# Banus/pano360

Hardware: AMD Instinct MI355X
Metric: blended megapixels/sec (multiband) (higher is better)
Workload: dtype f32; 1 GPU; cfg3: 32 synthetic 3840x2160 frames per image set, spherical warp + multiband blend L=5, native resolution (MAX_RESOLUTION uncapped); frames=32

## Files before the change

pano360_amd/csrc/blend.hip:

```cpp
#include <stdlib.h>

#include "geom.h"

__global__ __launch_bounds__(256) void ownership_kernel(
    const pano_patch *__restrict__ patches, int n, int H, int W,
    int16_t *__restrict__ owner, uint8_t *__restrict__ valid) {
    const int x = blockIdx.x * 64 + threadIdx.x, y = blockIdx.y * 4 + threadIdx.y;
    if (x >= W || y >= H) return;
    float best = 0.0f;
    int who = -1;
    bool any = false;
    for (int i = 0; i < n; ++i) {
        const pano_patch p = patches[i];
        const int px = x - p.x0, py = y - p.y0;
        if ((unsigned)px >= (unsigned)p.w || (unsigned)py >= (unsigned)p.h) continue;
        const float a = p.planes[3 * (size_t)p.vh * p.vpitch + (size_t)py * p.vpitch + px];
        if (a > best) {
            best = a;
            who = i;
        }
        any |= p.mask[(size_t)py * p.w + px] == 0;
    }
    owner[(size_t)y * W + x] = (int16_t)who;
    valid[(size_t)y * W + x] = any ? 1 : 0;
// ... 383 lines not shown
            s_rng[2] = lo_t; s_rng[3] = hi_t;
        }
        __syncthreads();
        const int tid = wave * 64 + lane;
        const bool keep = tid < listed && alpha_bound(cams + sh.list[tid], s_rng).hi >= 0.0f;
        const unsigned long long bal = __ballot(keep);
        if (lane == 0) s_kept[wave] = __popcll(bal);
        __syncthreads();
        int off = 0;
        for (int w = 0; w < wave; ++w) off += s_kept[w];
        off += __popcll(bal & ((1ull << lane) - 1ull));
        if (keep) s_keep[off] = sh.list[tid];
        ncand = s_kept[0] + s_kept[1] + s_kept[2] + s_kept[3];
        list = s_keep;
        __syncthreads();
    }

    const int x = bx0 + threadIdx.x, y = by0 + threadIdx.y;
    if (x >= xs1 || y >= H) return;
    const double s = sin_t[x], c = cos_t[x], t = tan_p[y];
    float acc[3] = {0.0f, 0.0f, 0.0f}, wsum = 0.0f;
    uint8_t last[3] = {0, 0, 0};
    bool any = false;
    for (int kk = 0; kk < ncand; ++kk) {
        const int k = LINEAR ? kk : ncand - 1 - kk;
        const int i = listed < 0 ? k : __builtin_amdgcn_readfirstlane(list[k]);
        const pano_camera *cam = cams + i;
        const int px = x - cam->x0, py = y - cam->y0;
        if ((unsigned)px >= (unsigned)cam->w || (unsigned)py >= (unsigned)cam->h) continue;
        float fx, fy;
        const int sw = cam->sw, sh_ = cam->sh;
        if (map_pixel(cam->proj, s, c, t, sw, sh_, fx, fy)) continue;
        any = true;
        const Taps tp = make_taps_unmasked(fx, fy, sw, sh_);
        const TapBytes tb = load_taps(cam->frame, sw, tp);
        float rgb[3];
        const float *__restrict__ gl = lut + (size_t)i * 256;
#pragma unroll
        for (int ch = 0; ch < 3; ++ch)
            rgb[ch] = PERCAM ? lerp4(lut_at(gl, tb.v[0][ch]), lut_at(gl, tb.v[1][ch]), lut_at(gl, tb.v[2][ch]),
                                     lut_at(gl, tb.v[3][ch]), tp)
                             : lerp4(lut_at(s_lut, tb.v[0][ch]), lut_at(s_lut, tb.v[1][ch]), lut_at(s_lut, tb.v[2][ch]),
                                     lut_at(s_lut, tb.v[3][ch]), tp);
        if (LINEAR) {
            const float a = alpha_at(cam->hat_x, cam->hat_y, tp);
#pragma unroll
            for (int ch = 0; ch < 3; ++ch) acc[ch] = acc[ch] + rgb[ch] * a;
            wsum = wsum + a;
        } else {
#pragma unroll
            for (int ch = 0; ch < 3; ++ch) last[ch] = (uint8_t)(int)(255.0f * rgb[ch]);
            break;
        }
    }
    const size_t g = ((size_t)y * W + x) * 3;
    if (LINEAR) {
        const float ws = wsum == 0.0f ? 1.0f : wsum;
#pragma unroll
        for (int ch = 0; ch < 3; ++ch)
            mosaic[g + ch] = (uint8_t)(int)(255.0f * __fdiv_rn(acc[ch], ws));
    } else {
        mosaic[g] = last[0];
        mosaic[g + 1] = last[1];
        mosaic[g + 2] = last[2];
    }
    if (valid) valid[(size_t)y * W + x] = any ? 1 : 0;
}

typedef short own8 __attribute__((ext_vector_type(8), aligned(2)));

__device__ __forceinline__ void owned_box_pixel(int o, int x, int y, bool up, bool down, bool left,
                                                bool right, int W, int32_t *__restrict__ boxes,
                                                int stride, uint8_t *__restrict__ marks) {
    if (o < 0) return;
    if (up && marks) marks[(size_t)o * W + x] = 1;
    if (!left && !right) return;
    if (left && up) {
        atomicMin(&boxes[(size_t)stride * o + 0], y);
        atomicMin(&boxes[(size_t)stride * o + 2], x);
    }
    if (left && down) atomicMax(&boxes[(size_t)stride * o + 1], y);
    if (right && up) atomicMax(&boxes[(size_t)stride * o + 3], x);
}

__global__ __launch_bounds__(256) void owned_boxes_kernel(const int16_t *__restrict__ owner,
                                                          int H, int W, int xs0, int xs1,
                                                          int32_t *__restrict__ boxes, int stride,
                                                          uint8_t *__restrict__ marks) {
    const int x8 = xs0 + (blockIdx.x * 64 + threadIdx.x) * 8, y = blockIdx.y * 4 + threadIdx.y;
    if (x8 >= xs1 || y >= H) return;
    const int16_t *row = owner + (size_t)y * W;
    const bool top = y == 0, bottom = y == H - 1;
    if (x8 + 8 <= xs1) {
        const own8 cur = *(const own8 *)(row + x8);
        const own8 upv = top ? cur : *(const own8 *)(row - W + x8);
        const own8 dnv = bottom ? cur : *(const own8 *)(row + W + x8);
        const int before = x8 == xs0 ? -32768 : row[x8 - 1];
        const int after = x8 + 8 == xs1 ? -32768 : row[x8 + 8];
#pragma unroll
        for (int j = 0; j < 8; ++j) {
            const int o = cur[j];
            const int l = j == 0 ? before : cur[j - 1], r = j == 7 ? after : cur[j + 1];
            owned_box_pixel(o, x8 + j, y, top || upv[j] != o, bottom || dnv[j] != o, l != o, r != o,
                            W, boxes, stride, marks);
        }
        return;
    }
    for (int x = x8; x < xs1; ++x) {
        const int o = row[x];
        owned_box_pixel(o, x, y, top || row[x - W] != o, bottom || row[x + W] != o,
                        x == xs0 || row[x - 1] != o, x == xs1 - 1 || row[x + 1] != o, W, boxes,
                        stride, marks);
    }
}

__device__ __forceinline__ uint8_t quant255(float v) { return (uint8_t)(int)(255.0f * v); }

#define IB PANO_INTERIOR_BLOCK

__global__ __launch_bounds__(256) void block_owner_kernel(const int16_t *__restrict__ owner,
                                                          int H, int W, int xs0, int xs1,
                                                          int H8, int W8, int blo, int bhi,
                                                          int16_t *__restrict__ bown) {
    const int bx = blo + blockIdx.x * 64 + threadIdx.x, by = blockIdx.y * 4 + threadIdx.y;
    if (bx >= bhi || by >= H8) return;
    const int x0 = bx * IB, y0 = by * IB;
    int o = -2;
    if (x0 >= xs0 && (x0 + IB < W ? x0 + IB : W) <= xs1) {
        o = owner[(size_t)y0 * W + x0];
        const bool whole = x0 + IB <= W && (W & 1) == 0;
        if (x0 + IB <= W && y0 + IB <= H) {
            static_assert(IB == 4, "one 8-byte load per block row");
            typedef uint64_t u64_any __attribute__((aligned(2)));
            const uint64_t o16 = (uint16_t)o;
            const uint64_t all = o16 | o16 << 16 | o16 << 32 | o16 << 48;
            uint64_t diff = 0;
#pragma unroll
            for (int dy = 0; dy < IB; ++dy)
                diff |= *(const u64_any *)(owner + (size_t)(y0 + dy) * W + x0) ^ all;
            if (diff) o = -2;
        } else
        for (int dy = 0; dy < IB && o != -2; ++dy) {
            const int y = y0 + dy;
            if (y >= H) break;
            if (whole) {
                const uint32_t *q = (const uint32_t *)(owner + (size_t)y * W + x0);
                const uint32_t both = ((uint32_t)(uint16_t)o << 16) | (uint16_t)o;
                uint32_t diff = 0;
#pragma unroll
                for (int k = 0; k < IB / 2; ++k) diff |= q[k] ^ both;
                if (diff) o = -2;
            } else {
                for (int dx = 0; dx < IB; ++dx) {
                    const int x = x0 + dx;
                    if (x >= W) break;
                    if (owner[(size_t)y * W + x] != o) {
                        o = -2;
                        break;
                    }
                }
            }
        }
    }
    bown[(size_t)by * W8 + bx] = (int16_t)o;
}

#define IT_W 64
#define IT_H 16
#define IT_REACH_MAX 20
__device__ __forceinline__ bool agree(int a, int b) { return a == b || a == -3 || b == -3; }

struct LevelReaches {
    int n;
    int reach[PANO_MAX_LEVELS];
};

__global__ __launch_bounds__(256) void interior_tile_kernel(const int16_t *__restrict__ bown,
                                                            int H8, int W8, int reach, int blo,
                                                            int bhi, int ilo, int ihi,
                                                            uint8_t *__restrict__ interior,
                                                            LevelReaches lv,
                                                            uint8_t *__restrict__ classes) {
    __shared__ int16_t s_own[(IT_H + 2 * IT_REACH_MAX) * (IT_W + 2 * IT_REACH_MAX)];
    __shared__ int16_t s_col[IT_H * (IT_W + 2 * IT_REACH_MAX)];
    __shared__ unsigned long long s_vmask[IT_W + 2 * IT_REACH_MAX];
    const int tid = threadIdx.x, lane = tid & 63, wave = tid >> 6;
    const int bx0 = ilo + blockIdx.x * IT_W, by0 = blockIdx.y * IT_H;
    const int tw = IT_W + 2 * reach, th = IT_H + 2 * reach;
    for (int ty = wave; ty < th; ty += 4) {
        const int y = by0 - reach + ty;
        const bool row_in = y >= 0 && y < H8;
        for (int tx = lane; tx < tw; tx += 64) {
            const int x = bx0 - reach + tx;
            s_own[ty * tw + tx] = (row_in && x >= 0 && x < W8)
                                      ? (x >= blo && x < bhi ? bown[(size_t)y * W8 + x] : (int16_t)-2)
                                      : (int16_t)-3;
        }
    }
    __syncthreads();
    for (int tx = tid; tx < tw; tx += 256) {
        unsigned long long m = 0;
        int prev = s_own[tx];
#pragma unroll 8
        for (int ty = 0; ty + 1 < th; ++ty) {
            const int cur = s_own[(ty + 1) * tw + tx];
            m |= (unsigned long long)agree(prev, cur) << ty;
            prev = cur;
        }
        s_vmask[tx] = m;
    }
    __syncthreads();
    int cls[IT_H / 4];
#pragma unroll
    for (int r = 0; r < IT_H / 4; ++r) cls[r] = 0;
    const int nlv = classes ? lv.n : 1;
    for (int q = 0; q < nlv; ++q) {
        const int rq = classes ? lv.reach[q] : reach, off = reach - rq;
        const unsigned long long full = (1ull << (2 * rq)) - 1ull;
        for (int ry = wave; ry < IT_H; ry += 4)
            for (int tx = lane; tx < tw; tx += 64) {
                const int o = s_own[(ry + reach) * tw + tx];
                const bool same = ((s_vmask[tx] >> (ry + off)) & full) == full;
                s_col[ry * tw + tx] = (int16_t)(o >= 0 && !same ? -2 : o);
            }
        __syncthreads();
#pragma unroll
        for (int r = 0; r < IT_H / 4; ++r) {
            const int ry = wave + 4 * r;
            const int16_t *row = s_col + ry * tw;
            const int a0 = row[lane], a1 = row[min(lane + 1, tw - 1)];
            const int b0 = row[min(lane + 64, tw - 1)], b1 = row[min(lane + 65, tw - 1)];
            const unsigned long long lo = __ballot(lane + 1 < tw && agree(a0, a1));
            const unsigned long long hi = __ballot(lane + 65 < tw && agree(b0, b1));
            const int sh = lane + off;
            const unsigned long long win = sh == 0 ? lo
                                           : sh < 64 ? (lo >> sh) | (hi << (64 - sh))
                                                     : hi >> (sh - 64);
            const int o = row[lane + reach];
            if (o >= 0 && (win & full) == full && cls[r] == q) cls[r] = q + 1;
        }
        __syncthreads();
    }
#pragma unroll
    for (int r = 0; r < IT_H / 4; ++r) {
        const int y = by0 + wave + 4 * r, x = bx0 + lane;
        if (y >= H8 || x >= ihi) continue;
        interior[(size_t)y * W8 + x] = cls[r] == nlv ? 1 : 0;
        if (classes) classes[(size_t)y * W8 + x] = (uint8_t)cls[r];
    }
}

struct InteriorArgs {
    const uint8_t *interior;
    int W8;
    const pano_camera *cams;
    const double *sin_t, *cos_t, *tan_p;
    const float *lut;
    const uint8_t *classes;
};

enum { LUT_LDS = 0, LUT_GLOBAL = 1 };

template <int LUT>
__device__ __forceinline__ void shade_interior(const pano_camera *cam, const float *__restrict__ table,
                                               const InteriorArgs &ia, int x, int y, int W,
                                               uint8_t *__restrict__ mosaic,
                                               float *__restrict__ mosaic_f32) {
    if (!cam->frame) return;
    const int sw = cam->sw, sh = cam->sh;
    float fx, fy;
    map_pixel(cam->proj, table_f64(ia.sin_t, x), table_f64(ia.cos_t, x), table_f64(ia.tan_p, y), sw, sh, fx, fy);
    Taps tp = tap_base(fx, fy);
    TapBytes tb;
    if (__ballot(!taps_interior(tp, sw, sh)) == 0ull) {
        tb = load_taps_interior(cam->frame, sw, tp);
    } else {
        tp.x1 = min(tp.x1, sw - 1);
        tp.y1 = min(tp.y1, sh - 1);
        tb = load_taps(cam->frame, sw, tp);
    }
    const size_t g = ((size_t)y * W + x) * 3;
#pragma unroll
    for (int c = 0; c < 3; ++c) {
        float v = lerp4(lut_at(table, tb.v[0][c]), lut_at(table, tb.v[1][c]),
                        lut_at(table, tb.v[2][c]), lut_at(table, tb.v[3][c]), tp);
        v = v < 0.0f ? 0.0f : (v > 1.0f ? 1.0f : v);
        if (mosaic_f32) mosaic_f32[g + c] = v;
        mosaic[g + c] = (uint8_t)(int)(255.0f * v);
    }
}

template <int LUT>
__device__ __forceinline__ void shade_interior_of(int own, const float *__restrict__ table, int stride,
                                                  const InteriorArgs &ia, int x, int y, int W,
                                                  uint8_t *__restrict__ mosaic,
                                                  float *__restrict__ mosaic_f32) {
    const int own_u = __builtin_amdgcn_readfirstlane(own);
    if (__ballot(own != own_u) == 0)
        shade_interior<LUT>(ia.cams + own_u, table + (size_t)own_u * stride, ia, x, y, W, mosaic, mosaic_f32);
    else
        shade_interior<LUT>(ia.cams + own, table + (size_t)own * stride, ia, x, y, W, mosaic, mosaic_f32);
}

#define COMPOSE_MASKS 4
template <int L, bool PERCAM, bool CLS>
__global__ __launch_bounds__(256) void multiband_compose_kernel(
    const pano_patch *__restrict__ patches, int n, int H, int W, int xs0, int xs1,
    const int16_t *__restrict__ owner, const uint8_t *__restrict__ valid,
    uint8_t *__restrict__ mosaic, float *__restrict__ mosaic_f32, InteriorArgs ia) {
    __shared__ float s_lut[256];
    if (ia.interior && !PERCAM) {
        s_lut[threadIdx.y * 64 + threadIdx.x] = ia.lut[threadIdx.y * 64 + threadIdx.x];
        __syncthreads();
    }
    const int x = xs0 + blockIdx.x * 64 + threadIdx.x, y = blockIdx.y * 4 + threadIdx.y;
    const bool inside = x < xs1 && y < H;
    const bool is_interior = inside && ia.interior && ia.interior[(size_t)(y / IB) * ia.W8 + x / IB];
    unsigned long long cand[COMPOSE_MASKS] = {};
    const bool masked = n <= 64 * COMPOSE_MASKS && __ballot(inside && !is_interior) != 0;
    if (masked) {
        const int wx0 = xs0 + blockIdx.x * 64, wx1 = min(wx0 + 64, xs1);
#pragma unroll
        for (int m = 0; m < COMPOSE_MASKS; ++m) {
            const int i = 64 * m + (int)threadIdx.x;
            bool hit = false;
            if (i < n) {
                const pano_patch *q = patches + i;
                const int ax = q->x0 + q->ax0, ay = q->y0 + q->ay0;
                hit = ax < wx1 && ax + q->aw > wx0 && ay <= y && y < ay + q->ah;
            }
            cand[m] = __ballot(hit);
        }
    }
    if (!inside) return;
    if (is_interior) {
        const int own = owner[(size_t)y * W + x];
        if (PERCAM)
            shade_interior_of<LUT_GLOBAL>(own, ia.lut, 256, ia, x, y, W, mosaic, mosaic_f32);
        else
            shade_interior_of<LUT_LDS>(own, s_lut, 0, ia, x, y, W, mosaic, mosaic_f32);
        return;
    }
    float layer[L][3], wsum[L];
#pragma unroll
    for (int k = 0; k < L; ++k) layer[k][0] = layer[k][1] = layer[k][2] = wsum[k] = 0.0f;
    const int j = CLS && L > 1 ? (int)ia.classes[(size_t)(y / IB) * ia.W8 + x / IB] : 0;
    const int own_px = CLS && j > 0 ? (int)owner[(size_t)y * W + x] : -1;
    float base[3] = {0.0f, 0.0f, 0.0f};

    int m = 0;
    unsigned long long bits = masked ? cand[0] : 0ull;
    for (int i = 0;; ++i) {
        if (masked) {
            while (bits == 0ull && ++m < COMPOSE_MASKS) bits = cand[m];
            if (bits == 0ull) break;
            i = 64 * m + __ffsll((long long)bits) - 1;
            bits &= bits - 1ull;
        } else if (i >= n) {
            break;
        }
        const pano_patch p = patches[i];
        const int ax = x - p.x0 - p.ax0, ay = y - p.y0 - p.ay0;
        if ((unsigned)ax >= (unsigned)p.aw || (unsigned)ay >= (unsigned)p.ah) continue;
        const size_t vplane = (size_t)p.vh * p.vpitch;
        const size_t vo = (size_t)(ay + p.ay0 - p.vy0) * p.vpitch + (ax + p.ax0 - p.vx0);
        const size_t aplane = (size_t)p.ah * p.apitch, ao = (size_t)ay * p.apitch + ax;
        float hi[3], ha = 0.0f;
        if (!CLS || j == 0) {
#pragma unroll
            for (int c = 0; c < 3; ++c) hi[c] = p.planes[c * vplane + vo];
        } else {
            const float *b = p.blurred + (size_t)(j - 1) * 4 * aplane + ao;
#pragma unroll
            for (int c = 0; c < 3; ++c) hi[c] = b[c * aplane];
            if (p.index == own_px) {
#pragma unroll
                for (int c = 0; c < 3; ++c) base[c] = p.planes[c * vplane + vo] - hi[c];
            }
        }
        if (L == 1) ha = owner[(size_t)y * W + x] == p.index ? 1.0f : 0.0f;
#pragma unroll
        for (int k = 0; k < L; ++k) {
            if (CLS && k < j) continue;
            float rgb[3], a;
            if (k < L - 1) {
                const float *b = p.blurred + (size_t)k * 4 * aplane + ao;
                a = b[3 * aplane];
#pragma unroll
                for (int c = 0; c < 3; ++c) {
                    const float g = b[c * aplane];
                    rgb[c] = hi[c] - g;
                    hi[c] = g;
                }
                ha = a;
            } else {
                a = ha;
#pragma unroll
                for (int c = 0; c < 3; ++c) rgb[c] = hi[c];
            }
#pragma unroll
            for (int c = 0; c < 3; ++c) layer[k][c] = layer[k][c] + rgb[c] * a;
            wsum[k] = wsum[k] + a;
        }
    }
    const bool ok = valid[(size_t)y * W + x] != 0;
    float out[3] = {CLS && ok ? base[0] : 0.0f, CLS && ok ? base[1] : 0.0f, CLS && ok ? base[2] : 0.0f};
#pragma unroll
    for (int k = 0; k < L; ++k) {
        if (CLS && k < j) continue;
        const float ws = wsum[k] == 0.0f ? 1.0f : wsum[k];
#pragma unroll
        for (int c = 0; c < 3; ++c)
            out[c] = out[c] + __fdiv_rn(ok ? layer[k][c] : 0.0f, ws);
    }
    const size_t g = ((size_t)y * W + x) * 3;
#pragma unroll
    for (int c = 0; c < 3; ++c) {
        float v = out[c];
        v = v < 0.0f ? 0.0f : (v > 1.0f ? 1.0f : v);
        if (mosaic_f32) mosaic_f32[g + c] = v;
        mosaic[g + c] = quant255(v);
    }
}

__global__ __launch_bounds__(256) void linear_blend_kernel(
    const pano_patch *__restrict__ patches, int n, int H, int W,
    uint8_t *__restrict__ mosaic) {
    const int x = blockIdx.x * 64 + threadIdx.x, y = blockIdx.y * 4 + threadIdx.y;
    if (x >= W || y >= H) return;
    float acc[3] = {0.0f, 0.0f, 0.0f}, wsum = 0.0f;
    for (int i = 0; i < n; ++i) {
        const pano_patch p = patches[i];
        const int px = x - p.x0, py = y - p.y0;
        if ((unsigned)px >= (unsigned)p.w || (unsigned)py >= (unsigned)p.h) continue;
        const size_t plane = (size_t)p.vh * p.vpitch, o = (size_t)py * p.vpitch + px;
        const bool m = p.mask[(size_t)py * p.w + px] != 0;
        const float a = p.planes[3 * plane + o];
#pragma unroll
        for (int c = 0; c < 3; ++c) {
            const float t = m ? 0.0f : p.planes[c * plane + o];
            acc[c] = acc[c] + t * a;
        }
        wsum = wsum + a;
    }
    const float ws = wsum == 0.0f ? 1.0f : wsum;
    const size_t g = ((size_t)y * W + x) * 3;
#pragma unroll
    for (int c = 0; c < 3; ++c) mosaic[g + c] = quant255(__fdiv_rn(acc[c], ws));
}

__global__ __launch_bounds__(256) void no_blend_kernel(
    const pano_patch *__restrict__ patches, int n, int H, int W,
    uint8_t *__restrict__ mosaic) {
    const int x = blockIdx.x * 64 + threadIdx.x, y = blockIdx.y * 4 + threadIdx.y;
    if (x >= W || y >= H) return;
    uint8_t out[3] = {0, 0, 0};
    for (int i = 0; i < n; ++i) {
        const pano_patch p = patches[i];
        const int px = x - p.x0, py = y - p.y0;
        if ((unsigned)px >= (unsigned)p.w || (unsigned)py >= (unsigned)p.h) continue;
        if (p.mask[(size_t)py * p.w + px]) continue;
        const size_t plane = (size_t)p.vh * p.vpitch, o = (size_t)py * p.vpitch + px;
#pragma unroll
        for (int c = 0; c < 3; ++c) out[c] = quant255(p.planes[c * plane + o]);
    }
    const size_t g = ((size_t)y * W + x) * 3;
    mosaic[g] = out[0];
    mosaic[g + 1] = out[1];
    mosaic[g + 2] = out[2];
}

static int check_table(const void *table, int n, int H, int W, const char *who) {
    PANO_REQUIRE(table, "%s: null table", who);
    PANO_REQUIRE(n >= 0 && n <= 32767, "%s: %d patches (int16 owner map holds 32767)", who, n);
    PANO_REQUIRE(H > 0 && W > 0, "%s: bad mosaic shape %dx%d", who, H, W);
    return PANO_OK;
}

#define MOSAIC_GRID dim3 block(64, 4), grid(ceil_div(W, 64), ceil_div(H, 4))

extern "C" int pano_ownership(pano_ctx *ctx, const pano_patch *patches, int n, int H, int W,
                              int16_t *owner, uint8_t *valid) {
    PANO_ENTER(ctx, "pano_ownership");
    if (int rc = check_table(patches, n, H, W, "pano_ownership")) return rc;
    PANO_REQUIRE(owner && valid, "pano_ownership: null output");
    MOSAIC_GRID;
    PANO_TIMED(PK_OWNERSHIP, (hipStream_t)stream,
               hipLaunchKernelGGL(ownership_kernel, grid, block, 0, (hipStream_t)stream,
                                  patches, n, H, W, owner, valid));
    PANO_LAUNCH_CHECK("ownership_kernel");
    return PANO_OK;
}

extern "C" int pano_ownership_cameras(pano_ctx *ctx, const pano_camera *cams, int n, int H, int W,
                                      int xs0, int xs1, const double *sin_t, const double *cos_t,
                                      const double *tan_p, int16_t *owner, uint8_t *valid) {
    PANO_ENTER(ctx, "pano_ownership_cameras");
    if (int rc = check_table(cams, n, H, W, "pano_ownership_cameras")) return rc;
    PANO_REQUIRE(sin_t && cos_t && tan_p && owner && valid, "pano_ownership_cameras: null pointer");
    PANO_REQUIRE(xs0 >= 0 && xs1 <= W && xs0 <= xs1, "pano_ownership_cameras: bad strip [%d, %d)", xs0, xs1);
    if (xs0 == xs1) return PANO_OK;
    const int prune = ctx->opt[PANO_OPT_OWN_PRUNE];
    dim3 block(64, 4), grid(ceil_div(xs1 - xs0, 64), ceil_div(H, (prune & 2) ? OWN_TILE_ROWS : OW_TH_TALL));
    PANO_TIMED(PK_OWNERSHIP_CAMS, (hipStream_t)stream,
               hipLaunchKernelGGL((prune & 2) ? ownership_cameras_l1_kernel : ownership_cameras_kernel,
                                  grid, block, (prune & 2) ? 0 : own_shared_bytes(n),
                                  (hipStream_t)stream, cams, n, H, W, xs0, xs1, sin_t, cos_t,
                                  tan_p, owner, valid, prune & 1, (int32_t *)nullptr, 0,
                                  (uint8_t *)nullptr));
    PANO_LAUNCH_CHECK("ownership_cameras_kernel");
    return PANO_OK;
}

extern "C" int pano_blend_cameras(pano_ctx *ctx, const pano_camera *cams, int n, int H, int W,
                                  int xs0, int xs1, int linear, const double *sin_t,
                                  const double *cos_t, const double *tan_p, const float *lut,
                                  int lut_stride, uint8_t *mosaic, uint8_t *valid) {
    PANO_ENTER(ctx, "pano_blend_cameras");
    if (int rc = check_table(cams, n, H, W, "pano_blend_cameras")) return rc;
    PANO_REQUIRE(sin_t && cos_t && tan_p && lut && mosaic, "pano_blend_cameras: null pointer");
    PANO_REQUIRE(lut_stride == 0 || lut_stride == 256,
                 "pano_blend_cameras: lut_stride %d (0 = shared table, 256 = per camera)", lut_stride);
    PANO_REQUIRE(xs0 >= 0 && xs1 <= W && xs0 <= xs1, "pano_blend_cameras: bad strip [%d, %d)", xs0, xs1);
    if (xs0 == xs1) return PANO_OK;
    dim3 block(64, 4), grid(ceil_div(xs1 - xs0, 64), ceil_div(H, 4));
    hipStream_t s = (hipStream_t)stream;
#define BLEND(LIN, PC)                                                                        \
    PANO_TIMED(PK_BLEND_CAMERAS, s,                                                           \
               hipLaunchKernelGGL((blend_cameras_kernel<LIN, PC>), grid, block, 0, s, cams, n, \
                                  H, W, xs0, xs1, sin_t, cos_t, tan_p, lut, mosaic, valid))
    if (linear && lut_stride) BLEND(true, true);
    else if (linear) BLEND(true, false);
    else if (lut_stride) BLEND(false, true);
    else BLEND(false, false);
#undef BLEND
    PANO_LAUNCH_CHECK("blend_cameras_kernel");
    return PANO_OK;
}

#define SPAN_WORDS 1024
__global__ __launch_bounds__(256) void owned_spans_kernel(const uint8_t *__restrict__ marks,
                                                          int W, int xs0, int xs1, int min_gap,
                                                          int max_spans, int stride,
                                                          int32_t *__restrict__ regions) {
    __shared__ unsigned long long s_bits[SPAN_WORDS];
    const int lane = threadIdx.x & 63, wave = threadIdx.x >> 6;
    const uint8_t *row = marks + (size_t)blockIdx.x * W;
    int32_t *out = regions + (size_t)blockIdx.x * stride + 5;
    int cnt = 0, last = 0;
    const int32_t *box = regions + (size_t)blockIdx.x * stride;
    xs0 = max(xs0, box[2]);
    xs1 = min(xs1, box[3] + 1);
    for (int chunk0 = xs0; chunk0 < xs1; chunk0 += 64 * SPAN_WORDS) {
        const int words = min(SPAN_WORDS, (xs1 - chunk0 + 63) >> 6);
        for (int w = wave; w < words; w += 4) {
            const int x = chunk0 + 64 * w + lane;
            const unsigned long long bal = __ballot(x < xs1 && row[x] != 0);
            if (lane == 0) s_bits[w] = bal;
        }
        __syncthreads();
        if (wave == 0) {
            for (int w = 0; w < words; ++w) {
                const int base = chunk0 + 64 * w;
                unsigned long long bal = s_bits[w];
                while (bal) {
                    const int s = __ffsll((long long)bal) - 1;
                    const unsigned long long rest = ~(bal >> s);
                    const int len = rest ? __ffsll((long long)rest) - 1 : 64 - s;
                    const int xa = base + s, xb = xa + len - 1;
                    if (cnt && (xa - last - 1 < min_gap || cnt == max_spans)) {
                        if (lane == 0) out[2 * (cnt - 1) + 1] = xb;
                    } else {
                        if (lane == 0) {
                            out[2 * cnt] = xa;
                            out[2 * cnt + 1] = xb;
                        }
                        ++cnt;
                    }
                    last = xb;
                    bal = s + len >= 64 ? 0ull : bal & ~((1ull << (s + len)) - 1ull);
                }
            }
        }
        __syncthreads();
    }
    if (threadIdx.x == 0) regions[(size_t)blockIdx.x * stride + 4] = cnt;
}

__global__ __launch_bounds__(256) void init_regions_kernel(int32_t *regions, int n, int stride,
                                                           uint8_t *marks, size_t mark_bytes) {
    const size_t i = (size_t)blockIdx.x * 256 + threadIdx.x;
    if (i < (size_t)n) {
        int32_t *r = regions + i * stride;
        r[0] = 0x7fffffff;
        r[1] = -1;
        r[2] = 0x7fffffff;
        r[3] = -1;
        r[4] = 0;
    }
    const size_t words = mark_bytes / 16, step = (size_t)gridDim.x * 256;
    uint4 *m16 = (uint4 *)marks;
    for (size_t k = i; k < words; k += step) m16[k] = make_uint4(0u, 0u, 0u, 0u);
    if (i < mark_bytes - words * 16) marks[words * 16 + i] = 0;
}

static int launch_init_regions(hipStream_t s, int32_t *regions, int n, int stride, uint8_t *marks,
                               int W) {
    size_t bytes = (size_t)n * W;
    if ((uintptr_t)marks & 15) {
        PANO_HIP(hipMemsetAsync(marks, 0, bytes, s));
        bytes = 0;
    }
    const size_t want = bytes / 16 / 256 + 1;
    const int blocks = (int)(want < 2048 ? (want > (size_t)ceil_div(n, 256) ? want : ceil_div(n, 256))
                                         : 2048);
    hipLaunchKernelGGL(init_regions_kernel, dim3(blocks), dim3(256), 0, s, regions, n, stride, marks,
                       bytes);
    PANO_LAUNCH_CHECK("init_regions_kernel");
    return PANO_OK;
}

extern "C" int pano_owned_regions(pano_ctx *ctx, const int16_t *owner, int H, int W, int xs0,
                                  int xs1, int n, int min_gap, int max_spans, uint8_t *marks,
                                  int32_t *regions) {
    PANO_ENTER(ctx, "pano_owned_regions");
    PANO_REQUIRE(owner && marks && regions, "pano_owned_regions: null pointer");
    PANO_REQUIRE(H > 0 && W > 0 && n >= 0 && n <= 32767 && max_spans >= 1 && min_gap >= 0,
                 "pano_owned_regions: bad argument");
    PANO_REQUIRE(xs0 >= 0 && xs1 <= W && xs0 <= xs1, "pano_owned_regions: bad strip [%d, %d)", xs0, xs1);
    if (n == 0) return PANO_OK;
    hipStream_t s = (hipStream_t)stream;
    const int stride = 5 + 2 * max_spans;
    if (int rc = launch_init_regions(s, regions, n, stride, marks, W)) return rc;
    if (xs0 == xs1) return PANO_OK;
    dim3 block(64, 4), grid(ceil_div(xs1 - xs0, 512), ceil_div(H, 4));
    PANO_TIMED(PK_OWNED_BOXES, s,
               hipLaunchKernelGGL(owned_boxes_kernel, grid, block, 0, s, owner, H, W, xs0, xs1,
                                  regions, stride, marks));
    PANO_LAUNCH_CHECK("owned_boxes_kernel");
    PANO_TIMED(PK_OWNED_SPANS, s,
               hipLaunchKernelGGL(owned_spans_kernel, dim3(n), dim3(256), 0, s, marks, W, xs0, xs1,
                                  min_gap, max_spans, stride, regions));
    PANO_LAUNCH_CHECK("owned_spans_kernel");
    return PANO_OK;
}

extern "C" int pano_ownership_regions(pano_ctx *ctx, const pano_camera *cams, int n, int H, int W,
                                      int xs0, int xs1, const double *sin_t, const double *cos_t,
                                      const double *tan_p, int16_t *owner, uint8_t *valid,
                                      int min_gap, int max_spans, uint8_t *marks,
                                      int32_t *regions) {
    PANO_ENTER(ctx, "pano_ownership_regions");
    if (int rc = check_table(cams, n, H, W, "pano_ownership_regions")) return rc;
    PANO_REQUIRE(sin_t && cos_t && tan_p && owner && valid && marks && regions,
                 "pano_ownership_regions: null pointer");
    PANO_REQUIRE(xs0 >= 0 && xs1 <= W && xs0 <= xs1, "pano_ownership_regions: bad strip [%d, %d)", xs0, xs1);
    PANO_REQUIRE(max_spans >= 1 && min_gap >= 0, "pano_ownership_regions: bad argument");
    if (n == 0) return PANO_OK;
    hipStream_t s = (hipStream_t)stream;
    const int stride = 5 + 2 * max_spans;
    if (int rc = launch_init_regions(s, regions, n, stride, marks, W)) return rc;
    if (xs0 == xs1) return PANO_OK;
    const int prune = ctx->opt[PANO_OPT_OWN_PRUNE];
    dim3 block(64, 4), grid(ceil_div(xs1 - xs0, 64), ceil_div(H, (prune & 2) ? OWN_TILE_ROWS : OW_TH_TALL));
    PANO_TIMED(PK_OWNERSHIP_CAMS, s,
               hipLaunchKernelGGL((prune & 2) ? ownership_cameras_l1_kernel : ownership_cameras_kernel,
                                  grid, block, (prune & 2) ? 0 : own_shared_bytes(n), s, cams, n, H, W, xs0,
                                  xs1, sin_t, cos_t, tan_p, owner, valid, prune & 1, regions, stride,
                                  marks));
    PANO_LAUNCH_CHECK("ownership_cameras_kernel");
    PANO_TIMED(PK_OWNED_SPANS, s,
               hipLaunchKernelGGL(owned_spans_kernel, dim3(n), dim3(256), 0, s, marks, W, xs0, xs1,
                                  min_gap, max_spans, stride, regions));
    PANO_LAUNCH_CHECK("owned_spans_kernel");
    return PANO_OK;
}

static int interior_map_launch(pano_ctx *ctx, const int16_t *owner, int H, int W, int xs0, int xs1,
                               const int *radii, int n_radii, int16_t *block_owner,
                               uint8_t *interior, uint8_t *classes, const char *who) {
    void *const stream = (void *)ctx->stream;
    PANO_REQUIRE(owner && block_owner && interior && radii, "%s: null pointer", who);
    PANO_REQUIRE(H > 0 && W > 0 && n_radii >= 1 && n_radii < PANO_MAX_LEVELS, "%s: bad argument", who);
    PANO_REQUIRE(xs0 >= 0 && xs1 <= W && xs0 <= xs1, "%s: bad strip [%d, %d)", who, xs0, xs1);
    LevelReaches lv = {};
    lv.n = n_radii;
    for (int k = 0; k < n_radii; ++k) {
        PANO_REQUIRE(radii[k] >= 0 && (k == 0 || radii[k] >= radii[k - 1]),
                     "%s: radii must ascend (level %d: %d)", who, k, radii[k]);
        lv.reach[k] = ceil_div(radii[k] + IB - 1, IB);
    }
    const int radius = radii[n_radii - 1];
    const int H8 = ceil_div(H, IB), W8 = ceil_div(W, IB), reach = lv.reach[n_radii - 1];
    if (xs0 == xs1) return PANO_OK;
    const int ilo = xs0 / IB, ihi = ceil_div(xs1, IB);
    const int blo = ilo - reach > 0 ? ilo - reach : 0, bhi = ihi + reach < W8 ? ihi + reach : W8;
    dim3 block(64, 4), grid(ceil_div(bhi - blo, 64), ceil_div(H8, 4));
    hipStream_t s = (hipStream_t)stream;
    PANO_TIMED(PK_INTERIOR, s,
               hipLaunchKernelGGL(block_owner_kernel, grid, block, 0, s, owner, H, W, xs0, xs1,
                                  H8, W8, blo, bhi, block_owner));
    PANO_LAUNCH_CHECK("block_owner_kernel");
    PANO_REQUIRE(reach <= IT_REACH_MAX, "%s: radius %d reaches %d blocks (at most %d)", who, radius,
                 reach, IT_REACH_MAX);
    hipLaunchKernelGGL(interior_tile_kernel, dim3(ceil_div(ihi - ilo, IT_W), ceil_div(H8, IT_H)),
                       dim3(256), 0, s, block_owner, H8, W8, reach, blo, bhi, ilo, ihi, interior, lv,
                       classes);
    PANO_LAUNCH_CHECK("interior_tile_kernel");
    return PANO_OK;
}

extern "C" int pano_interior_map(pano_ctx *ctx, const int16_t *owner, int H, int W, int xs0,
                                 int xs1, int radius, int16_t *block_owner, uint8_t *interior) {
    PANO_ENTER(ctx, "pano_interior_map");
    return interior_map_launch(ctx, owner, H, W, xs0, xs1, &radius, 1, block_owner, interior, nullptr,
                               "pano_interior_map");
}

extern "C" int pano_interior_classes(pano_ctx *ctx, const int16_t *owner, int H, int W, int xs0,
                                     int xs1, const int *radii, int n_radii, int16_t *block_owner,
                                     uint8_t *interior, uint8_t *classes) {
    PANO_ENTER(ctx, "pano_interior_classes");
    PANO_REQUIRE(classes, "pano_interior_classes: null pointer");
    return interior_map_launch(ctx, owner, H, W, xs0, xs1, radii, n_radii, block_owner, interior,
                               classes, "pano_interior_classes");
}

extern "C" int pano_multiband_compose(pano_ctx *ctx, const pano_patch *patches, int n, int H,
                                      int W, int xs0, int xs1, int n_levels, const int16_t *owner,
                                      const uint8_t *valid, const uint8_t *interior,
                                      const uint8_t *classes, const pano_camera *cams,
                                      const double *sin_t,
                                      const double *cos_t, const double *tan_p, const float *lut,
                                      int lut_stride, uint8_t *mosaic, float *mosaic_f32) {
    PANO_ENTER(ctx, "pano_multiband_compose");
    if (int rc = check_table(patches, n, H, W, "pano_multiband_compose")) return rc;
    PANO_REQUIRE(H > 0 && W > 0, "pano_multiband_compose: bad mosaic shape %dx%d", H, W);
    PANO_REQUIRE(owner && mosaic && valid, "pano_multiband_compose: null pointer");
    PANO_REQUIRE(n_levels >= 1 && n_levels <= PANO_MAX_LEVELS,
                 "pano_multiband_compose: n_levels %d outside [1, %d]", n_levels, PANO_MAX_LEVELS);
    PANO_REQUIRE(xs0 >= 0 && xs1 <= W && xs0 <= xs1,
                 "pano_multiband_compose: bad strip [%d, %d)", xs0, xs1);
    PANO_REQUIRE(!interior || (cams && sin_t && cos_t && tan_p && lut),
                 "pano_multiband_compose: the interior map needs cameras, tables and LUT");
    PANO_REQUIRE(lut_stride == 0 || lut_stride == 256,
                 "pano_multiband_compose: lut_stride %d (0 = shared table, 256 = per camera)",
                 lut_stride);
    if (xs0 == xs1) return PANO_OK;
    PANO_REQUIRE(!classes || interior, "pano_multiband_compose: level classes without the interior map");
    InteriorArgs ia = {interior, ceil_div(W, IB), cams, sin_t, cos_t, tan_p, lut,
                       ctx->opt[PANO_OPT_LEVEL_CLASSES] ? classes : nullptr};
    const bool percam = interior && lut_stride != 0;
    dim3 block(64, 4), grid(ceil_div(xs1 - xs0, 64), ceil_div(H, 4));
    hipStream_t s = (hipStream_t)stream;
#define COMPOSE_AS(L, PC, CL)                                                            \
    PANO_TIMED(PK_COMPOSE, s,                                                           \
               hipLaunchKernelGGL((multiband_compose_kernel<L, PC, CL>), grid, block, 0, s, \
                                  patches, n, H, W, xs0, xs1, owner, valid, mosaic,     \
                                  mosaic_f32, ia))
#define COMPOSE(L)                                                                      \
    case L:                                                                             \
        if (ia.classes && L > 1) {                                                      \
            if (percam) COMPOSE_AS(L, true, true); else COMPOSE_AS(L, false, true);     \
        } else {                                                                        \
            if (percam) COMPOSE_AS(L, true, false); else COMPOSE_AS(L, false, false);   \
        }                                                                               \
        break;
    switch (n_levels) {
        COMPOSE(1) COMPOSE(2) COMPOSE(3) COMPOSE(4) COMPOSE(5) COMPOSE(6) COMPOSE(7) COMPOSE(8)
    }
#undef COMPOSE_AS
#undef COMPOSE
    PANO_LAUNCH_CHECK("multiband_compose_kernel");
    return PANO_OK;
}

extern "C" int pano_linear_blend(pano_ctx *ctx, const pano_patch *patches, int n, int H, int W,
                                 uint8_t *mosaic) {
    PANO_ENTER(ctx, "pano_linear_blend");
    if (int rc = check_table(patches, n, H, W, "pano_linear_blend")) return rc;
    PANO_REQUIRE(mosaic, "pano_linear_blend: null output");
    MOSAIC_GRID;
    PANO_TIMED(PK_LINEAR, (hipStream_t)stream,
               hipLaunchKernelGGL(linear_blend_kernel, grid, block, 0, (hipStream_t)stream,
                                  patches, n, H, W, mosaic));
    PANO_LAUNCH_CHECK("linear_blend_kernel");
    return PANO_OK;
}

extern "C" int pano_no_blend(pano_ctx *ctx, const pano_patch *patches, int n, int H, int W,
                             uint8_t *mosaic) {
    PANO_ENTER(ctx, "pano_no_blend");
    if (int rc = check_table(patches, n, H, W, "pano_no_blend")) return rc;
    PANO_REQUIRE(mosaic, "pano_no_blend: null output");
    MOSAIC_GRID;
    PANO_TIMED(PK_NOBLEND, (hipStream_t)stream,
               hipLaunchKernelGGL(no_blend_kernel, grid, block, 0, (hipStream_t)stream,
                                  patches, n, H, W, mosaic));
    PANO_LAUNCH_CHECK("no_blend_kernel");
    return PANO_OK;
}
```

Before: 209,900 MP/s.

## Process four rows per thread in multiband compose, batching interior shading

The compose kernel now has each thread cover four rows spaced four apart, so the grid is four times shorter. Per-column sin/cos values and the camera projection matrix are loaded once and reused across the rows, and the interior bilinear taps are issued in batches of two rows to overlap memory latency. Seam pixels fall through to a refactored per-pixel path, and the candidate patch mask now covers the taller block. Launch bounds gain a minimum-waves hint that depends on the level count. The costs are higher register pressure, more patch candidates per block and fewer blocks for the scheduler to spread.

```diff
diff --git a/pano360_amd/csrc/blend.hip b/pano360_amd/csrc/blend.hip
--- a/pano360_amd/csrc/blend.hip
+++ b/pano360_amd/csrc/blend.hip
@@ -709,45 +709,85 @@
         shade_interior<LUT>(ia.cams + own, table + (size_t)own * stride, ia, x, y, W, mosaic, mosaic_f32);
 }
 
+#define COMPOSE_ROWS 4
+
+template <int LUT, int J0, int NR>
+__device__ __forceinline__ void shade_interior_rows(const pano_camera *cam, const float *__restrict__ table,
+                                                    double s, double c, const double *__restrict__ tan_p, int H,
+                                                    unsigned live, int x, int y0, int W,
+                                                    uint8_t *__restrict__ mosaic,
+                                                    float *__restrict__ mosaic_f32) {
+    typedef const __attribute__((address_space(4))) pano_camera *cam_ptr;
+    const cam_ptr cc = (cam_ptr)cam;
+    const uint8_t *const frame = cc->frame;
+    if (!frame) return;
+    const int sw = cc->sw, sh = cc->sh;
+    double K[9];
+#pragma unroll
+    for (int i = 0; i < 9; ++i) K[i] = cc->proj[i];
+    double t[COMPOSE_ROWS];
+#pragma unroll
+    for (int j = J0; j < J0 + NR; ++j) t[j] = table_f64(tan_p, min(y0 + 4 * j, H - 1));
+    Taps tp[COMPOSE_ROWS];
+    TapBytes tb[COMPOSE_ROWS];
+    bool inner = true;
+#pragma unroll
+    for (int j = J0; j < J0 + NR; ++j) {
+        float fx, fy;
+        map_pixel(K, s, c, t[j], sw, sh, fx, fy);
+        if (!((live >> j) & 1u)) fx = fy = 0.0f;
+        tp[j] = tap_base(fx, fy);
+        inner &= taps_interior(tp[j], sw, sh);
+    }
+    if (__ballot(!inner) == 0ull) {
+#pragma unroll
+        for (int j = J0; j < J0 + NR; ++j) tb[j] = load_taps_interior(frame, sw, tp[j]);
+    } else {
+#pragma unroll
+        for (int j = J0; j < J0 + NR; ++j) {
+            tp[j].x1 = min(tp[j].x1, sw - 1);
+            tp[j].y1 = min(tp[j].y1, sh - 1);
+            tb[j] = load_taps(frame, sw, tp[j]);
+        }
+    }
+#pragma unroll
+    for (int j = J0; j < J0 + NR; ++j) {
+        if (!((live >> j) & 1u)) continue;
+        const size_t g = ((size_t)(y0 + 4 * j) * W + x) * 3;
+#pragma unroll
+        for (int ch = 0; ch < 3; ++ch) {
+            float v = lerp4(lut_at(table, tb[j].v[0][ch]), lut_at(table, tb[j].v[1][ch]),
+                            lut_at(table, tb[j].v[2][ch]), lut_at(table, tb[j].v[3][ch]), tp[j]);
+            v = v < 0.0f ? 0.0f : (v > 1.0f ? 1.0f : v);
+            if (mosaic_f32) mosaic_f32[g + ch] = v;
+            mosaic[g + ch] = (uint8_t)(int)(255.0f * v);
+        }
+    }
+}
+
+#define COMPOSE_BATCH 2
+template <int LUT>
+__device__ __forceinline__ void shade_interior_batches(const pano_camera *cam, const float *__restrict__ table,
+                                                       double s, double c, const double *__restrict__ tan_p, int H,
+                                                       unsigned live, int x, int y0, int W,
+                                                       uint8_t *__restrict__ mosaic,
+                                                       float *__restrict__ mosaic_f32) {
+    shade_interior_rows<LUT, 0, COMPOSE_BATCH>(cam, table, s, c, tan_p, H, live, x, y0, W, mosaic, mosaic_f32);
+    if (COMPOSE_BATCH < COMPOSE_ROWS)
+        shade_interior_rows<LUT, COMPOSE_ROWS - COMPOSE_BATCH, COMPOSE_BATCH>(cam, table, s, c, tan_p, H, live, x,
+                                                                             y0,
+                                                                             W, mosaic, mosaic_f32);
+}
+
+#define COMPOSE_WAVES(L, CLS) ((L) + ((CLS) && (L) >= 5) <= 5 ? 8 : (L) + ((CLS) && (L) >= 5) == 6 ? 7 : (L) + ((CLS) && (L) >= 5) == 7 ? 6 : 5)
 #define COMPOSE_MASKS 4
-template <int L, bool PERCAM, bool CLS>
-__global__ __launch_bounds__(256) void multiband_compose_kernel(
-    const pano_patch *__restrict__ patches, int n, int H, int W, int xs0, int xs1,
-    const int16_t *__restrict__ owner, const uint8_t *__restrict__ valid,
-    uint8_t *__restrict__ mosaic, float *__restrict__ mosaic_f32, InteriorArgs ia) {
-    __shared__ float s_lut[256];
-    if (ia.interior && !PERCAM) {
-        s_lut[threadIdx.y * 64 + threadIdx.x] = ia.lut[threadIdx.y * 64 + threadIdx.x];
-        __syncthreads();
-    }
-    const int x = xs0 + blockIdx.x * 64 + threadIdx.x, y = blockIdx.y * 4 + threadIdx.y;
-    const bool inside = x < xs1 && y < H;
-    const bool is_interior = inside && ia.interior && ia.interior[(size_t)(y / IB) * ia.W8 + x / IB];
-    unsigned long long cand[COMPOSE_MASKS] = {};
-    const bool masked = n <= 64 * COMPOSE_MASKS && __ballot(inside && !is_interior) != 0;
-    if (masked) {
-        const int wx0 = xs0 + blockIdx.x * 64, wx1 = min(wx0 + 64, xs1);
-#pragma unroll
-        for (int m = 0; m < COMPOSE_MASKS; ++m) {
-            const int i = 64 * m + (int)threadIdx.x;
-            bool hit = false;
-            if (i < n) {
-                const pano_patch *q = patches + i;
-                const int ax = q->x0 + q->ax0, ay = q->y0 + q->ay0;
-                hit = ax < wx1 && ax + q->aw > wx0 && ay <= y && y < ay + q->ah;
-            }
-            cand[m] = __ballot(hit);
-        }
-    }
-    if (!inside) return;
-    if (is_interior) {
-        const int own = owner[(size_t)y * W + x];
-        if (PERCAM)
-            shade_interior_of<LUT_GLOBAL>(own, ia.lut, 256, ia, x, y, W, mosaic, mosaic_f32);
-        else
-            shade_interior_of<LUT_LDS>(own, s_lut, 0, ia, x, y, W, mosaic, mosaic_f32);
-        return;
-    }
+
+template <int L, bool CLS>
+__device__ __forceinline__ void compose_seam_pixel(
+    const pano_patch *__restrict__ patches, int n, int W, int x, int y, bool masked,
+    const unsigned long long (&cand)[COMPOSE_MASKS], const int16_t *__restrict__ owner,
+    const uint8_t *__restrict__ valid, uint8_t *__restrict__ mosaic, float *__restrict__ mosaic_f32,
+    const InteriorArgs &ia) {
     float layer[L][3], wsum[L];
 #pragma unroll
     for (int k = 0; k < L; ++k) layer[k][0] = layer[k][1] = layer[k][2] = wsum[k] = 0.0f;
@@ -827,6 +867,92 @@
         v = v < 0.0f ? 0.0f : (v > 1.0f ? 1.0f : v);
         if (mosaic_f32) mosaic_f32[g + c] = v;
         mosaic[g + c] = quant255(v);
+    }
+}
+
+template <int L, bool PERCAM, bool CLS>
+__global__ __launch_bounds__(256, COMPOSE_WAVES(L, CLS)) void multiband_compose_kernel(
+    const pano_patch *__restrict__ patches, int n, int H, int W, int xs0, int xs1,
+    const int16_t *__restrict__ owner, const uint8_t *__restrict__ valid,
+    uint8_t *__restrict__ mosaic, float *__restrict__ mosaic_f32, InteriorArgs ia) {
+    __shared__ float s_lut[256];
+    constexpr int BH = 4 * COMPOSE_ROWS;
+    const int x = xs0 + blockIdx.x * 64 + threadIdx.x, y0 = blockIdx.y * BH + threadIdx.y;
+    const bool col_in = x < xs1;
+    if (ia.interior && !PERCAM) s_lut[threadIdx.y * 64 + threadIdx.x] = ia.lut[threadIdx.y * 64 + threadIdx.x];
+    unsigned inter = 0u, seam = 0u;
+#pragma unroll
+    for (int j = 0; j < COMPOSE_ROWS; ++j) {
+        const int y = y0 + 4 * j;
+        const bool inside = col_in && y < H;
+        const bool it = inside && ia.interior && ia.interior[(size_t)(y / IB) * ia.W8 + x / IB];
+        inter |= (it ? 1u : 0u) << j;
+        seam |= (inside && !it ? 1u : 0u) << j;
+    }
+    int own[COMPOSE_ROWS] = {};
+    double sn = 0.0, cs = 0.0;
+    if (ia.interior) {
+        const int xc = min(x, xs1 - 1);
+        sn = table_f64(ia.sin_t, xc);
+        cs = table_f64(ia.cos_t, xc);
+#pragma unroll
+        for (int j = 0; j < COMPOSE_ROWS; ++j) {
+            const int yc = min(y0 + 4 * j, H - 1);
+            own[j] = owner[(size_t)yc * W + xc];
+        }
+        if (!PERCAM) __syncthreads();
+    }
+    unsigned long long cand[COMPOSE_MASKS] = {};
+    const bool masked = n <= 64 * COMPOSE_MASKS && __ballot(seam != 0u) != 0ull;
+    if (masked) {
+        const int wx0 = xs0 + blockIdx.x * 64, wx1 = min(wx0 + 64, xs1);
+        const int wy1 = min(y0 + 4 * (COMPOSE_ROWS - 1), H - 1);
+#pragma unroll
+        for (int m = 0; m < COMPOSE_MASKS; ++m) {
+            const int i = 64 * m + (int)threadIdx.x;
+            bool hit = false;
+            if (i < n) {
+                const pano_patch *q = patches + i;
+                const int ax = q->x0 + q->ax0, ay = q->y0 + q->ay0;
+                hit = ax < wx1 && ax + q->aw > wx0 && ay <= wy1 && y0 < ay + q->ah;
+            }
+            cand[m] = __ballot(hit);
+        }
+    }
+    if (inter) {
+        int o = own[0];
+#pragma unroll
+        for (int j = 1; j < COMPOSE_ROWS; ++j) o = (inter >> j) & 1u ? own[j] : o;
+        const int own_u = __builtin_amdgcn_readfirstlane(o);
+        bool same = true;
+#pragma unroll
+        for (int j = 0; j < COMPOSE_ROWS; ++j) same &= !((inter >> j) & 1u) || own[j] == own_u;
+        if (__ballot(!same) == 0ull) {
+            const pano_camera *cam = ia.cams + own_u;
+            if (PERCAM)
+                shade_interior_batches<LUT_GLOBAL>(cam, ia.lut + (size_t)own_u * 256, sn, cs, ia.tan_p, H, inter, x,
+                                                   y0, W, mosaic, mosaic_f32);
+            else
+                shade_interior_batches<LUT_LDS>(cam, s_lut, sn, cs, ia.tan_p, H, inter, x, y0, W, mosaic, mosaic_f32);
+        } else {
+#pragma unroll 1
+            for (int j = 0; j < COMPOSE_ROWS; ++j) {
+                if (!((inter >> j) & 1u)) continue;
+                const int y = y0 + 4 * j, own_px = owner[(size_t)y * W + x];
+                if (PERCAM)
+                    shade_interior_of<LUT_GLOBAL>(own_px, ia.lut, 256, ia, x, y, W, mosaic, mosaic_f32);
+                else
+                    shade_interior_of<LUT_LDS>(own_px, s_lut, 0, ia, x, y, W, mosaic, mosaic_f32);
+            }
+        }
+    }
+#pragma unroll 1
+    for (int j = 0; j < COMPOSE_ROWS; ++j) {
+        const bool mine = (seam >> j) & 1u;
+        if (__ballot(mine) == 0ull) continue;
+        if (mine)
+            compose_seam_pixel<L, CLS>(patches, n, W, x, y0 + 4 * j, masked, cand, owner, valid, mosaic,
+                                       mosaic_f32, ia);
     }
 }
 
@@ -1158,7 +1284,7 @@
     InteriorArgs ia = {interior, ceil_div(W, IB), cams, sin_t, cos_t, tan_p, lut,
                        ctx->opt[PANO_OPT_LEVEL_CLASSES] ? classes : nullptr};
     const bool percam = interior && lut_stride != 0;
-    dim3 block(64, 4), grid(ceil_div(xs1 - xs0, 64), ceil_div(H, 4));
+    dim3 block(64, 4), grid(ceil_div(xs1 - xs0, 64), ceil_div(H, 4 * COMPOSE_ROWS));
     hipStream_t s = (hipStream_t)stream;
 #define COMPOSE_AS(L, PC, CL)                                                            \
     PANO_TIMED(PK_COMPOSE, s,                                                           \
```

Result: faster. 221,900 MP/s, median of 6 (+5.7%).
